# interactiveaudiolab/ppgs

Measured on AMD Instinct MI355X. Metric: PPG frames/sec (whole node), mel repr, batch=32x1000 frames, higher is better.
Workload: dtype bf16; 1 GPU; configs[1]: mel representation, batch=32 x 1000 frames per GPU, audio resident in HBM -> (32,40,1000) fp32 posteriors in HBM; batch=32, frames=1000, per_gpu_batches=1, parallelism=utterance-sharded x1, no data-path collective

## Files before the change

### ppgs_amd/csrc/ppg_frontend.hip

```cpp
#include "ppg_lds.h"
#include "ppg_launch.h"

#include <hip/hip_fp16.h>

namespace {

constexpr int NFFT = 1024;
constexpr int HOP = 160;
constexpr int NBINS = 513;
constexpr int NMELS = 80;
constexpr int PADR = (NFFT - HOP) / 2;
constexpr int FPB = ppg::kFrontendFrames;
constexpr int SEG = NFFT + (FPB - 1) * HOP;
constexpr int BUF = NFFT + NFFT / 16;
constexpr int MSEG = ppg::kMelSegment;
constexpr int NS = ppg::kMelSteps;
constexpr int MROW = 1088;
__device__ __forceinline__ int sigma(int c) { return (0x6c >> (2 * c)) & 3; }

constexpr int OFF_TW = 0;
constexpr int SEGP = (SEG + 255) / 256 * 256;
constexpr int OFF_SEG = OFF_TW + 64 * 8;
constexpr int OFF_FFT = OFF_SEG + 2 * SEGP * 4;
constexpr int OFF_MAG = OFF_FFT + 4 * BUF * 8;
constexpr int LDS_BYTES = OFF_MAG + FPB * MROW;
constexpr int TEAMS = 2;
constexpr int CU_LDS_BYTES = 163840;
static_assert(2 * LDS_BYTES <= CU_LDS_BYTES && LDS_BYTES % 16 == 0, "two teams per CU; a two-team workgroup = the CU's LDS");
static_assert(OFF_MAG % 16 == 0 && MROW % 16 == 0, "fragment reads are 16-byte aligned");

typedef float cplx __attribute__((ext_vector_type(2)));
__device__ __forceinline__ cplx cadd(cplx a, cplx b) { return a + b; }
__device__ __forceinline__ cplx csub(cplx a, cplx b) { return a - b; }
__device__ __forceinline__ cplx cadd_mi(cplx a, cplx b) {
    cplx r;
    asm("v_pk_add_f32 %0, %1, %2 op_sel:[1,0] op_sel_hi:[0,1] neg_hi:[1,0]" : "=v"(r) : "v"(b), "v"(a));
    return r;
}
__device__ __forceinline__ cplx csub_mi(cplx a, cplx b) {
    cplx r;
    asm("v_pk_add_f32 %0, %1, %2 op_sel:[1,0] op_sel_hi:[0,1] neg_lo:[1,0]" : "=v"(r) : "v"(b), "v"(a));
    return r;
}
__device__ __forceinline__ cplx cmul(cplx a, cplx w) {
    cplx t, r;
    asm("v_pk_mul_f32 %0, %1, %2 op_sel:[0,0] op_sel_hi:[0,1]" : "=v"(t) : "v"(a), "v"(w));
    asm("v_fma_f32 %0, -%1, %2, %3" : "=v"(r.x) : "v"(a.y), "v"(w.y), "v"(t.x));
    asm("v_fma_f32 %0, %1, %2, %3" : "=v"(r.y) : "v"(a.y), "v"(w.x), "v"(t.y));
    return r;
}

template <bool CMI = false>
__device__ __forceinline__ void radix4(cplx& A, cplx& B, cplx& C, cplx& D) {
    const cplx apc = CMI ? cadd_mi(A, C) : cadd(A, C), amc = CMI ? csub_mi(A, C) : csub(A, C);
    const cplx bpd = cadd(B, D), bmd = csub(B, D);
    A = cadd(apc, bpd);
    B = cadd_mi(amc, bmd);
    C = csub(apc, bpd);
    D = csub_mi(amc, bmd);
}

template <int M>
__device__ __forceinline__ cplx w16() {
    constexpr float c1 = 0.92387953251128674f, s1 = 0.38268343236508977f, r = 0.70710678118654752f;
    if constexpr (M == 1) return cplx{c1, -s1};
    else if constexpr (M == 2) return cplx{r, -r};
    else if constexpr (M == 3) return cplx{s1, -c1};
    else if constexpr (M == 6) return cplx{-r, -r};
    else { static_assert(M == 9, "exponent"); return cplx{-c1, s1}; }
}

__device__ __forceinline__ void dft16(cplx (&x)[16]) {
#pragma unroll
    for (int r = 0; r < 4; ++r) radix4(x[r], x[r + 4], x[r + 8], x[r + 12]);
    x[5] = cmul(x[5], w16<1>());  x[9] = cmul(x[9], w16<2>());   x[13] = cmul(x[13], w16<3>());
    x[6] = cmul(x[6], w16<2>());   x[14] = cmul(x[14], w16<6>());
    x[7] = cmul(x[7], w16<3>());  x[11] = cmul(x[11], w16<6>()); x[15] = cmul(x[15], w16<9>());
    radix4(x[0], x[1], x[2], x[3]);
    radix4(x[4], x[5], x[6], x[7]);
    radix4<true>(x[8], x[9], x[10], x[11]);
    radix4(x[12], x[13], x[14], x[15]);
    cplx t;
#define PPG_SWAP(a, b) t = x[a]; x[a] = x[b]; x[b] = t;
    PPG_SWAP(1, 4) PPG_SWAP(2, 8) PPG_SWAP(3, 12) PPG_SWAP(6, 9) PPG_SWAP(7, 13) PPG_SWAP(11, 14)
#undef PPG_SWAP
}

__device__ __forceinline__ int pad(int i) { return i + (i >> 4); }

__device__ __forceinline__ void wave_sync() {
    asm volatile("s_waitcnt lgkmcnt(0)" ::: "memory");
    __builtin_amdgcn_fence(__ATOMIC_ACQ_REL, "wavefront");
    __builtin_amdgcn_wave_barrier();
}

template <bool SPEC, class SRC>
__device__ __forceinline__ void frontend_body(
    const ppg::FrontendTables& tb, const SRC& src, int total_groups, int wide_ok, __half* __restrict__ spec, __half* __restrict__ mel)
{
    extern __shared__ __attribute__((aligned(16))) char smem_all[];
    const int team = TEAMS == 1 ? 0 : __builtin_amdgcn_readfirstlane((int)(threadIdx.x >> 8));
    char* smem = smem_all + team * LDS_BYTES;
    cplx* tw = reinterpret_cast<cplx*>(smem + OFF_TW);
    float* seg0 = reinterpret_cast<float*>(smem + OFF_SEG);

    const int tid = threadIdx.x & 255;
    const int lane = tid & 63;
    const int wave = __builtin_amdgcn_readfirstlane(tid >> 6);
    cplx* buf = reinterpret_cast<cplx*>(smem + OFF_FFT) + wave * BUF;

    if (tid < 64) { const float2 w = tb.twiddle[16 * tid]; tw[tid] = cplx{w.x, w.y}; }
    reinterpret_cast<uint32_t*>(smem + OFF_MAG + (tid >> 4) * MROW + 1024)[tid & 15] = 0u;

    float hreg[16];
    cplx t1[16];
#pragma unroll
    for (int j = 0; j < 16; ++j) hreg[j] = tb.hann[lane + 64 * j];
#pragma unroll
    for (int k = 1; k < 16; ++k) { const float2 w = tb.twiddle[lane * k]; t1[k] = cplx{w.x, w.y}; }

    int step_frag[NS], step_off[NS], step_block[NS];
#pragma unroll
    for (int i = 0; i < NS; ++i) {
        const int4 e = tb.mel_prog[wave * NS + i];
        step_frag[i] = __builtin_amdgcn_readfirstlane(e.x);
        step_off[i] = __builtin_amdgcn_readfirstlane(e.y);
        step_block[i] = __builtin_amdgcn_readfirstlane(e.z);
    }

    auto stage = [&](int grp, int into) { src.stage(tb, grp, into, seg0, wave, lane, wide_ok); };
    const int stride = TEAMS * gridDim.x;
    const int first_group = TEAMS * blockIdx.x + team;
    if (first_group < total_groups) stage(first_group, 0);
    asm volatile("s_waitcnt vmcnt(0)" ::: "memory");

#ifdef PPG_FE_TIMING
    int stamp_group = 0;
    auto stamp = [&](int k) {
        if (tb.dbg && blockIdx.x == 0 && lane == 0 && stamp_group == 2) tb.dbg[wave * 16 + k] = __builtin_amdgcn_s_memtime();
    };
#else
    auto stamp = [&](int) {};
#endif
    int half = 0;
    const int trips = (total_groups - TEAMS * (int)blockIdx.x + stride - 1) / stride;
    int grp = first_group;
    for (int trip = 0; trip < trips; ++trip, grp += stride, half ^= 1) {
        const bool active = grp < total_groups;
        int b, f0, frames;
        src.group(grp, active, b, f0, frames);
        const float* seg = seg0 + half * SEGP;
        int pitch = src.pitch(frames);
        asm volatile("" : "+s"(pitch));
#ifdef PPG_FE_TIMING
        ++stamp_group;
#endif
        stamp(0);
        __syncthreads();
        stamp(1);

        auto transform = [&](const int j, const bool verify = false) {
            const int fa = f0 + 2 * j;
            if (fa >= frames) return;
            cplx x[16];
            {
                const float* sa = seg + (2 * j) * HOP + lane;
#pragma unroll
                for (int i = 0; i < 16; ++i) {
                    x[i] = cplx{sa[64 * i], sa[64 * i + HOP]} * hreg[i];
                }
                dft16(x);
#pragma unroll
                for (int k = 1; k < 16; ++k) x[k] = cmul(x[k], t1[k]);
#pragma unroll
                for (int k = 0; k < 16; ++k) buf[17 * lane + k] = x[k];
            }
            wave_sync();
            const int p0 = lane + (lane >> 4);
            {
#pragma unroll
                for (int i = 0; i < 16; ++i) x[i] = buf[p0 + 68 * i];
                dft16(x);
                const int p = lane >> 4, q = lane & 15;
#pragma unroll
                for (int k = 1; k < 16; ++k) x[k] = cmul(x[k], tw[p * k]);
                cplx* dst = buf + q + 272 * p;
#pragma unroll
                for (int k = 0; k < 16; ++k) dst[17 * k] = x[k];
            }
            wave_sync();
#pragma unroll
            for (int m = 0; m < 4; ++m) {
                cplx* z = buf + p0 + 68 * m;
                cplx A = z[0], B = z[272], C = z[544], D = z[816];
                radix4(A, B, C, D);
                z[0] = A; z[272] = B; z[544] = C; z[816] = D;
            }
            wave_sync();
            const int nb = (NFFT - lane) + ((NFFT - lane) >> 4);
            const int odd = lane & 1;
            const int row = j + 8 * odd;
            char* wdst = smem + OFF_MAG + row * MROW + ((((lane >> 3) ^ sigma(row >> 2)) << 2) + ((lane >> 1) & 3)) * 4;
            const uint32_t sel = odd ? 0x07060302u : 0x01000504u;
            auto split_bin = [&](int r, __half& ha, __half& hb) {
                const int k = lane + 64 * r;
                const cplx zk = buf[p0 + 68 * r];
                const cplx zn = buf[(r == 0 && lane == 0) ? 0 : nb - 68 * r];
                const float ar = 0.5f * (zk.x + zn.x), ai = 0.5f * (zk.y - zn.y);
                const float br = 0.5f * (zk.y + zn.y), bi = -0.5f * (zk.x - zn.x);
                ha = __float2half_rn(__builtin_amdgcn_sqrtf(ar * ar + ai * ai + 1e-6f));
                hb = __float2half_rn(__builtin_amdgcn_sqrtf(br * br + bi * bi + 1e-6f));
                if constexpr (SPEC) {
                    if (verify) return;
                    spec[(uint32_t)(b * NBINS + k) * (uint32_t)pitch + (uint32_t)fa] = ha;
                    if (fa + 1 < frames) spec[(uint32_t)(b * NBINS + k) * (uint32_t)pitch + (uint32_t)fa + 1u] = hb;
                }
            };
#pragma unroll
            for (int r = 0; r < 8; ++r) {
                __half ha, hb;
                split_bin(r, ha, hb);
                const uint32_t pk = (uint32_t)__half_as_ushort(ha) | ((uint32_t)__half_as_ushort(hb) << 16);
                const uint32_t other = (uint32_t)__builtin_amdgcn_mov_dpp((int)pk, 0xB1, 0xf, 0xf, true);
                const uint32_t val = __builtin_amdgcn_perm(pk, other, sel);
                *reinterpret_cast<uint32_t*>(wdst + 128 * r) = val;
            }
            if (verify) return;
            if (lane == 0) {
                __half ha, hb;
                split_bin(8, ha, hb);
                *reinterpret_cast<uint32_t*>(smem + OFF_MAG + j * MROW + ((64 ^ sigma(j >> 2)) << 4)) = __half_as_ushort(ha);
                *reinterpret_cast<uint32_t*>(smem + OFF_MAG + (j + 8) * MROW + ((64 ^ sigma((j + 8) >> 2)) << 4)) = __half_as_ushort(hb);
            }
        };

        transform(wave);
        stamp(2);
        if (!(wide_ok & 4) && grp + stride < total_groups) stage(grp + stride, half ^ 1);
        stamp(3);
        transform(wave + 4);
        stamp(4);
        u32x4 whi[NS], wlo[NS];
        asm volatile("s_waitcnt vmcnt(0)" ::: "memory");
        if (mel) {
            uint32_t loff = lane * 16;
            asm volatile("" : "+v"(loff));
#pragma unroll
            for (int i = 0; i < NS; ++i) {
                const char* src = reinterpret_cast<const char*>(tb.mel_img) + (size_t)step_frag[i] * 1024;
                whi[i] = *reinterpret_cast<const u32x4*>(src + loff);
                wlo[i] = *reinterpret_cast<const u32x4*>(src + 1024 + loff);
            }
        }
        __syncthreads();
        stamp(5);
        if (mel) {
            const int n = lane & 15, g = lane >> 4;
            const char* brow = smem + OFF_MAG + n * MROW + ((g ^ sigma(n >> 2)) << 4);
            f32x4 acc = {0.f, 0.f, 0.f, 0.f};
            const int frame = f0 + (n < 8 ? 2 * n : 2 * (n - 8) + 1);
#pragma unroll
            for (int i = 0; i < NS; ++i) {
                const u32x4 bfi = *reinterpret_cast<const u32x4*>(brow + step_off[i]);
                PrecF16::mma(acc, whi[i], bfi);
                PrecF16::mma(acc, wlo[i], bfi);
                const int block = step_block[i];
                if ((i == MSEG - 1 || i == NS - 1) && block >= 0) {
                    if (frame < frames) {
#pragma unroll
                        for (int e = 0; e < 4; ++e) {
                            const int m = 16 * block + 4 * g + e;
                            mel[(uint32_t)(b * NMELS + m) * (uint32_t)pitch + (uint32_t)frame] =
                                __float2half_rn(logf(fmaxf(acc[e] * (1.0f / 65536.0f), 1e-5f)));
                        }
                    }
                    acc = f32x4{0.f, 0.f, 0.f, 0.f};
                }
            }
        }
        stamp(6);
        if (wide_ok & 4) {
            __syncthreads();
            if (grp + stride < total_groups) stage(grp + stride, half ^ 1);
            asm volatile("s_waitcnt vmcnt(0)" ::: "memory");
        }
        if constexpr (SRC::kCarry) { if (active) src.carry_forward(grp, tid); }
    }
}

struct BatchSource {
    static constexpr bool kCarry = false;
    const float* __restrict__ audio;
    int samples, frames, groups_per_row;
    __device__ __forceinline__ void group(int grp, bool active, int& b, int& f0, int& nframes) const {
        b = active ? grp / groups_per_row : 0;
        f0 = active ? (grp - b * groups_per_row) * FPB : frames;
        nframes = frames;
    }
    __device__ __forceinline__ int pitch(int nframes) const { return nframes; }
    __device__ __forceinline__ void stage(const ppg::FrontendTables& tb, int grp, int into, float* seg0, int wave, int lane, int wide_ok) const {
        const int b = grp / groups_per_row;
        const int f0 = (grp - b * groups_per_row) * FPB;
        const float* arow = audio + (size_t)b * samples;
        const uint32_t dst = lds_addr(seg0) + into * (SEGP * 4);
        const int first = f0 * HOP - PADR;
        if ((wide_ok & 1) && first >= 0 && first + SEGP <= samples) {
#pragma unroll
            for (int j = 0; j < (SEGP / 256 + 3) / 4; ++j) {
                const int piece = wave + 4 * j;
                if (piece >= SEGP / 256) break;
                glds16_saddr(reinterpret_cast<const char*>(arow + first), (uint32_t)(piece * 1024 + lane * 16), dst + piece * 1024);
            }
            return;
        }
#pragma unroll 2
        for (int piece = wave; piece < SEGP / 64; piece += 4) {
            int src = first + piece * 64 + lane;
            if (src < 0) src = -src;
            if (src >= samples) src = 2 * (samples - 1) - src;
            const float* p = (src >= 0 && src < samples) ? arow + src : tb.hann;
            asm volatile("s_mov_b32 m0, %1\n\ts_nop 0\n\tglobal_load_lds_dword %0, off"
                         :: "v"(p), "s"(__builtin_amdgcn_readfirstlane(dst + piece * 256)) : "memory", "m0");
        }
    }
};

template <bool SPEC>
__global__ __launch_bounds__(256 * TEAMS, 2 / TEAMS) void frontend_kernel(
    ppg::FrontendTables tb, const float* __restrict__ audio, int samples, int frames,
    int groups_per_row, int total_groups, int wide_ok, __half* __restrict__ spec, __half* __restrict__ mel)
{
    frontend_body<SPEC>(tb, BatchSource{audio, samples, frames, groups_per_row}, total_groups, wide_ok, spec, mel);
}

struct StreamSource {
    static constexpr bool kCarry = true;
    ppg::FrontendStreamArgs a;
    __device__ __forceinline__ void group(int grp, bool active, int& b, int& f0, int& nframes) const {
        const int l = active ? grp / a.groups_per_item : 0;
        nframes = active ? a.item[l].frames : 0;
        f0 = active ? (grp - l * a.groups_per_item) * FPB : 0;
        b = a.item0 + l;
    }
    __device__ __forceinline__ int pitch(int) const { return a.out_pitch; }
    __device__ __forceinline__ const float* sample(const ppg::FrontendStreamItem& it, int l, int pos) const {
        return pos < it.split ? a.carry + ((size_t)(2 * (a.item0 + l) + it.cur) * a.cap + (pos - it.cbase))
                              : a.chunk + ((size_t)(a.item0 + l) * a.chunk_pitch + (pos - it.split));
    }
    __device__ __forceinline__ void stage(const ppg::FrontendTables& tb, int grp, int into, float* seg0, int wave, int lane, int) const {
        const int l = grp / a.groups_per_item;
        const int f0 = (grp - l * a.groups_per_item) * FPB;
        const ppg::FrontendStreamItem it = a.item[l];
        if (f0 >= it.frames) return;
        const uint32_t dst = lds_addr(seg0) + into * (SEGP * 4);
        const int first = f0 * HOP - PADR;
#pragma unroll 2
        for (int piece = wave; piece < SEGP / 64; piece += 4) {
            int pos = first + piece * 64 + lane;
            if (pos < it.lo) pos = 2 * it.lo - pos;
            if (pos >= it.hi) pos = 2 * (it.hi - 1) - pos;
            const float* p = (pos >= it.cbase && pos < it.hi) ? sample(it, l, pos) : tb.hann;
            asm volatile("s_mov_b32 m0, %1\n\ts_nop 0\n\tglobal_load_lds_dword %0, off"
                         :: "v"(p), "s"(__builtin_amdgcn_readfirstlane(dst + piece * 256)) : "memory", "m0");
        }
    }
    __device__ __forceinline__ void carry_forward(int grp, int tid) const {
        const int l = grp / a.groups_per_item;
        if (grp != l * a.groups_per_item) return;
        const ppg::FrontendStreamItem it = a.item[l];
        float* next = a.carry + (size_t)(2 * (a.item0 + l) + (it.cur ^ 1)) * a.cap;
        for (int pos = it.keep + tid; pos < it.hi; pos += 256) next[pos - it.keep] = *sample(it, l, pos);
    }
};

__global__ __launch_bounds__(256 * TEAMS, 2 / TEAMS) void frontend_stream_kernel(
    ppg::FrontendTables tb, StreamSource src, int total_groups, __half* __restrict__ mel)
{
    frontend_body<false>(tb, src, total_groups, 0, nullptr, mel);
}

}

namespace ppg {

hipError_t launch_frontend(const FrontendTables& tb, const float* audio, int batch, int samples,
                           void* spec, void* mel, hipStream_t s) {
    const int frames = samples / HOP;
    const int groups_per_row = (frames + FPB - 1) / FPB;
    if (mel && (!tb.mel_img || !tb.mel_prog)) return hipErrorInvalidValue;
    if ((double)batch * NBINS * frames >= 4294967296.0) return hipErrorInvalidValue;
    const int total = groups_per_row * batch;
    static LdsLimit limit[2];
    const void* kernel = spec ? reinterpret_cast<const void*>(frontend_kernel<true>) : reinterpret_cast<const void*>(frontend_kernel<false>);
    const hipError_t e = limit[spec != nullptr].ensure(kernel, CU_LDS_BYTES);
    if (e != hipSuccess) return e;
    static int slots = 0;
    if (slots == 0) {
        int dev = 0, cus = 0;
        if (hipGetDevice(&dev) != hipSuccess ||
            hipDeviceGetAttribute(&cus, hipDeviceAttributeMultiprocessorCount, dev) != hipSuccess || cus <= 0)
            cus = 256;
        slots = 2 * cus;
    }
    const int rounds = (total + slots - 1) / slots;
    const int teams = (total + rounds - 1) / rounds;
    const int grid = (teams + TEAMS - 1) / TEAMS;
    int wide_ok = (reinterpret_cast<uintptr_t>(audio) % 16 == 0 && samples % 4 == 0) ? 1 : 0;
    size_t lds_bytes = TEAMS == 2 ? CU_LDS_BYTES : LDS_BYTES;
    static const int fe_debug = env_experiment("PPGS_AMD_FE_DEBUG", 0);
    if (fe_debug & 1) wide_ok = 0;
    if (fe_debug & 4) wide_ok |= 4;
    if (fe_debug & 16) lds_bytes = TEAMS * LDS_BYTES;
    if (spec)
        hipLaunchKernelGGL(frontend_kernel<true>, dim3(grid), dim3(256 * TEAMS), lds_bytes, s, tb, audio, samples, frames,
                           groups_per_row, total, wide_ok, reinterpret_cast<__half*>(spec), reinterpret_cast<__half*>(mel));
    else
        hipLaunchKernelGGL(frontend_kernel<false>, dim3(grid), dim3(256 * TEAMS), lds_bytes, s, tb, audio, samples, frames,
                           groups_per_row, total, wide_ok, reinterpret_cast<__half*>(spec), reinterpret_cast<__half*>(mel));
    return hipGetLastError();
}

hipError_t launch_frontend_stream(const FrontendTables& tb, const FrontendStreamArgs& args, int items, void* mel, hipStream_t s) {
    if (!tb.mel_img || !tb.mel_prog || items <= 0 || items > kFrontendStreamItems || args.groups_per_item <= 0)
        return hipErrorInvalidValue;
    if ((double)(args.item0 + items) * NMELS * args.out_pitch >= 4294967296.0) return hipErrorInvalidValue;
    static LdsLimit limit;
    const hipError_t e = limit.ensure(reinterpret_cast<const void*>(frontend_stream_kernel), CU_LDS_BYTES);
    if (e != hipSuccess) return e;
    static int slots = 0;
    if (slots == 0) {
        int dev = 0, cus = 0;
        if (hipGetDevice(&dev) != hipSuccess ||
            hipDeviceGetAttribute(&cus, hipDeviceAttributeMultiprocessorCount, dev) != hipSuccess || cus <= 0)
            cus = 256;
        slots = 2 * cus;
    }
    const int total = args.groups_per_item * items;
    const int rounds = (total + slots - 1) / slots;
    const int teams = (total + rounds - 1) / rounds;
    const int grid = (teams + TEAMS - 1) / TEAMS;
    hipLaunchKernelGGL(frontend_stream_kernel, dim3(grid), dim3(256 * TEAMS), CU_LDS_BYTES, s, tb, StreamSource{args}, total,
                       reinterpret_cast<__half*>(mel));
    return hipGetLastError();
}

}
```

Before: 48.58 million frames/s.

## Restructure 1024-point FFT as 32x32 with half-wave transforms and bpermute spectrum split

Replaces the three-pass 16x16x4 FFT per wave with a two-pass 32x32 decomposition in which each half-wave (32 lanes) transforms one frame pair. The transpose goes through a float-wide padded LDS buffer in two halves (real, then imaginary), which halves the FFT scratch footprint. The conjugate-symmetric partner bins now come from ds_bpermute instead of LDS reads. Hann and twiddle values are loaded from global memory inside the loop rather than kept in registers, and the mel frame ordering changes to match the new row layout. This should cut LDS passes and barriers, but it raises register pressure with 32-element complex arrays and adds global reads on every trip.

```diff
diff --git a/ppgs_amd/csrc/ppg_frontend.hip b/ppgs_amd/csrc/ppg_frontend.hip
--- a/ppgs_amd/csrc/ppg_frontend.hip
+++ b/ppgs_amd/csrc/ppg_frontend.hip
@@ -2,6 +2,8 @@
 #include "ppg_launch.h"
 
 #include <hip/hip_fp16.h>
+
+#include <utility>
 
 namespace {
 
@@ -12,17 +14,17 @@
 constexpr int PADR = (NFFT - HOP) / 2;
 constexpr int FPB = ppg::kFrontendFrames;
 constexpr int SEG = NFFT + (FPB - 1) * HOP;
-constexpr int BUF = NFFT + NFFT / 16;
+constexpr int XROW = 33;
+constexpr int BUF = 2 * 32 * XROW;
 constexpr int MSEG = ppg::kMelSegment;
 constexpr int NS = ppg::kMelSteps;
 constexpr int MROW = 1088;
 __device__ __forceinline__ int sigma(int c) { return (0x6c >> (2 * c)) & 3; }
 
-constexpr int OFF_TW = 0;
 constexpr int SEGP = (SEG + 255) / 256 * 256;
-constexpr int OFF_SEG = OFF_TW + 64 * 8;
+constexpr int OFF_SEG = 0;
 constexpr int OFF_FFT = OFF_SEG + 2 * SEGP * 4;
-constexpr int OFF_MAG = OFF_FFT + 4 * BUF * 8;
+constexpr int OFF_MAG = OFF_FFT + 4 * BUF * 4;
 constexpr int LDS_BYTES = OFF_MAG + FPB * MROW;
 constexpr int TEAMS = 2;
 constexpr int CU_LDS_BYTES = 163840;
@@ -47,6 +49,13 @@
     asm("v_pk_mul_f32 %0, %1, %2 op_sel:[0,0] op_sel_hi:[0,1]" : "=v"(t) : "v"(a), "v"(w));
     asm("v_fma_f32 %0, -%1, %2, %3" : "=v"(r.x) : "v"(a.y), "v"(w.y), "v"(t.x));
     asm("v_fma_f32 %0, %1, %2, %3" : "=v"(r.y) : "v"(a.y), "v"(w.x), "v"(t.y));
+    return r;
+}
+__device__ __forceinline__ cplx cmul_conj(cplx a, cplx w) {
+    cplx t, r;
+    asm("v_pk_mul_f32 %0, %1, %2 op_sel:[0,0] op_sel_hi:[0,1]" : "=v"(t) : "v"(a), "v"(w));
+    asm("v_fma_f32 %0, %1, %2, %3" : "=v"(r.x) : "v"(a.y), "v"(w.y), "v"(t.x));
+    asm("v_fma_f32 %0, %1, %2, -%3" : "=v"(r.y) : "v"(a.y), "v"(w.x), "v"(t.y));
     return r;
 }
 
@@ -86,7 +95,30 @@
 #undef PPG_SWAP
 }
 
-__device__ __forceinline__ int pad(int i) { return i + (i >> 4); }
+template <int M>
+__device__ __forceinline__ cplx w32() {
+    constexpr float c[8] = {1.f, 0.98078528040323043f, 0.92387953251128674f, 0.83146961230254524f,
+                            0.70710678118654752f, 0.55557023301960218f, 0.38268343236508977f, 0.19509032201612825f};
+    static_assert(M >= 1 && M <= 7, "exponent");
+    return cplx{c[M], -c[8 - M]};
+}
+
+__device__ __forceinline__ void dft32(cplx (&x)[32]) {
+    cplx e[16], o[16];
+#pragma unroll
+    for (int i = 0; i < 16; ++i) { e[i] = x[2 * i]; o[i] = x[2 * i + 1]; }
+    dft16(e);
+    __builtin_amdgcn_sched_barrier(0);
+    dft16(o);
+    __builtin_amdgcn_sched_barrier(0);
+    auto fly = [&](auto kc) {
+        constexpr int k = decltype(kc)::value;
+        if constexpr (k % 8 != 0) o[k] = cmul(o[k], w32<k % 8>());
+        if constexpr (k < 8) { x[k] = cadd(e[k], o[k]); x[k + 16] = csub(e[k], o[k]); }
+        else { x[k] = cadd_mi(e[k], o[k]); x[k + 16] = csub_mi(e[k], o[k]); }
+    };
+    [&]<int... K>(std::integer_sequence<int, K...>) { (fly(std::integral_constant<int, K>{}), ...); }(std::make_integer_sequence<int, 16>{});
+}
 
 __device__ __forceinline__ void wave_sync() {
     asm volatile("s_waitcnt lgkmcnt(0)" ::: "memory");
@@ -101,23 +133,15 @@
     extern __shared__ __attribute__((aligned(16))) char smem_all[];
     const int team = TEAMS == 1 ? 0 : __builtin_amdgcn_readfirstlane((int)(threadIdx.x >> 8));
     char* smem = smem_all + team * LDS_BYTES;
-    cplx* tw = reinterpret_cast<cplx*>(smem + OFF_TW);
     float* seg0 = reinterpret_cast<float*>(smem + OFF_SEG);
 
     const int tid = threadIdx.x & 255;
     const int lane = tid & 63;
     const int wave = __builtin_amdgcn_readfirstlane(tid >> 6);
-    cplx* buf = reinterpret_cast<cplx*>(smem + OFF_FFT) + wave * BUF;
-
-    if (tid < 64) { const float2 w = tb.twiddle[16 * tid]; tw[tid] = cplx{w.x, w.y}; }
+    const int q = lane & 31, hw = lane >> 5;
+    float* xbuf = reinterpret_cast<float*>(smem + OFF_FFT) + wave * BUF + hw * (32 * XROW);
+
     reinterpret_cast<uint32_t*>(smem + OFF_MAG + (tid >> 4) * MROW + 1024)[tid & 15] = 0u;
-
-    float hreg[16];
-    cplx t1[16];
-#pragma unroll
-    for (int j = 0; j < 16; ++j) hreg[j] = tb.hann[lane + 64 * j];
-#pragma unroll
-    for (int k = 1; k < 16; ++k) { const float2 w = tb.twiddle[lane * k]; t1[k] = cplx{w.x, w.y}; }
 
     int step_frag[NS], step_off[NS], step_block[NS];
 #pragma unroll
@@ -159,86 +183,89 @@
         __syncthreads();
         stamp(1);
 
-        auto transform = [&](const int j, const bool verify = false) {
-            const int fa = f0 + 2 * j;
-            if (fa >= frames) return;
-            cplx x[16];
+
+        const bool work = f0 + 4 * wave < frames;
+        const int j = 2 * wave + hw;
+        const int fa = f0 + 2 * j;
+        cplx x[32];
+        if (work) {
             {
-                const float* sa = seg + (2 * j) * HOP + lane;
-#pragma unroll
-                for (int i = 0; i < 16; ++i) {
-                    x[i] = cplx{sa[64 * i], sa[64 * i + HOP]} * hreg[i];
-                }
-                dft16(x);
-#pragma unroll
-                for (int k = 1; k < 16; ++k) x[k] = cmul(x[k], t1[k]);
-#pragma unroll
-                for (int k = 0; k < 16; ++k) buf[17 * lane + k] = x[k];
-            }
-            wave_sync();
-            const int p0 = lane + (lane >> 4);
+                uint32_t qoff = q;
+                asm volatile("" : "+v"(qoff));
+                const float* hw_ = tb.hann + qoff;
+                const float* sa = seg + (2 * j) * HOP + q;
+#pragma unroll
+                for (int i = 0; i < 32; ++i) x[i] = cplx{sa[32 * i], sa[32 * i + HOP]} * hw_[32 * i];
+                cplx t1[17];
+#pragma unroll
+                for (int k = 1; k <= 16; ++k) { const float2 w = tb.twiddle[qoff * k]; t1[k] = cplx{w.x, w.y}; }
+                __builtin_amdgcn_sched_barrier(0);
+                dft32(x);
+                __builtin_amdgcn_sched_barrier(0);
+#pragma unroll
+                for (int k = 1; k < 32; ++k) x[k] = k <= 16 ? cmul(x[k], t1[k]) : cmul_conj(x[k], t1[32 - k]);
+            }
+        }
+        stamp(2);
+        if (!(wide_ok & 4) && grp + stride < total_groups) stage(grp + stride, half ^ 1);
+        if (work) {
             {
-#pragma unroll
-                for (int i = 0; i < 16; ++i) x[i] = buf[p0 + 68 * i];
-                dft16(x);
-                const int p = lane >> 4, q = lane & 15;
-#pragma unroll
-                for (int k = 1; k < 16; ++k) x[k] = cmul(x[k], tw[p * k]);
-                cplx* dst = buf + q + 272 * p;
-#pragma unroll
-                for (int k = 0; k < 16; ++k) dst[17 * k] = x[k];
-            }
-            wave_sync();
-#pragma unroll
-            for (int m = 0; m < 4; ++m) {
-                cplx* z = buf + p0 + 68 * m;
-                cplx A = z[0], B = z[272], C = z[544], D = z[816];
-                radix4(A, B, C, D);
-                z[0] = A; z[272] = B; z[544] = C; z[816] = D;
-            }
-            wave_sync();
-            const int nb = (NFFT - lane) + ((NFFT - lane) >> 4);
+                float* col = xbuf + XROW * q;
+                const float* rowp = xbuf + q;
+                float re[32];
+#pragma unroll
+                for (int k = 0; k < 32; ++k) col[k] = x[k].x;
+                wave_sync();
+#pragma unroll
+                for (int i = 0; i < 32; ++i) re[i] = rowp[XROW * i];
+                wave_sync();
+#pragma unroll
+                for (int k = 0; k < 32; ++k) col[k] = x[k].y;
+                wave_sync();
+#pragma unroll
+                for (int i = 0; i < 32; ++i) x[i] = cplx{re[i], rowp[XROW * i]};
+            }
+            stamp(3);
+            __builtin_amdgcn_sched_barrier(0);
+            dft32(x);
+            __builtin_amdgcn_sched_barrier(0);
             const int odd = lane & 1;
-            const int row = j + 8 * odd;
-            char* wdst = smem + OFF_MAG + row * MROW + ((((lane >> 3) ^ sigma(row >> 2)) << 2) + ((lane >> 1) & 3)) * 4;
+            const int row = 2 * j + odd;
+            char* wdst = smem + OFF_MAG + row * MROW + ((((q >> 3) ^ sigma(row >> 2)) << 2) + ((q >> 1) & 3)) * 4;
             const uint32_t sel = odd ? 0x07060302u : 0x01000504u;
-            auto split_bin = [&](int r, __half& ha, __half& hb) {
-                const int k = lane + 64 * r;
-                const cplx zk = buf[p0 + 68 * r];
-                const cplx zn = buf[(r == 0 && lane == 0) ? 0 : nb - 68 * r];
+            const int partner = ((lane & 32) | ((32 - q) & 31)) << 2;
+            auto split_bin = [&](int k, cplx zk, cplx zn, __half& ha, __half& hb) {
                 const float ar = 0.5f * (zk.x + zn.x), ai = 0.5f * (zk.y - zn.y);
                 const float br = 0.5f * (zk.y + zn.y), bi = -0.5f * (zk.x - zn.x);
                 ha = __float2half_rn(__builtin_amdgcn_sqrtf(ar * ar + ai * ai + 1e-6f));
                 hb = __float2half_rn(__builtin_amdgcn_sqrtf(br * br + bi * bi + 1e-6f));
                 if constexpr (SPEC) {
-                    if (verify) return;
-                    spec[(uint32_t)(b * NBINS + k) * (uint32_t)pitch + (uint32_t)fa] = ha;
+                    if (fa < frames) spec[(uint32_t)(b * NBINS + k) * (uint32_t)pitch + (uint32_t)fa] = ha;
                     if (fa + 1 < frames) spec[(uint32_t)(b * NBINS + k) * (uint32_t)pitch + (uint32_t)fa + 1u] = hb;
                 }
             };
 #pragma unroll
-            for (int r = 0; r < 8; ++r) {
+            for (int k2 = 0; k2 < 16; ++k2) {
+                const cplx mine = (q == 0 || q >= 17) ? x[(32 - k2) & 31] : x[31 - k2];
+                cplx zn;
+                zn.x = __int_as_float(__builtin_amdgcn_ds_bpermute(partner, __float_as_int(mine.x)));
+                zn.y = __int_as_float(__builtin_amdgcn_ds_bpermute(partner, __float_as_int(mine.y)));
                 __half ha, hb;
-                split_bin(r, ha, hb);
+                split_bin(q + 32 * k2, q >= 17 ? x[k2 + 1] : x[k2], zn, ha, hb);
                 const uint32_t pk = (uint32_t)__half_as_ushort(ha) | ((uint32_t)__half_as_ushort(hb) << 16);
                 const uint32_t other = (uint32_t)__builtin_amdgcn_mov_dpp((int)pk, 0xB1, 0xf, 0xf, true);
                 const uint32_t val = __builtin_amdgcn_perm(pk, other, sel);
-                *reinterpret_cast<uint32_t*>(wdst + 128 * r) = val;
-            }
-            if (verify) return;
-            if (lane == 0) {
+                *reinterpret_cast<uint32_t*>(wdst + 64 * k2) = val;
+                if (k2 % 4 == 3) __builtin_amdgcn_sched_barrier(0);
+            }
+            if (q == 0) {
                 __half ha, hb;
-                split_bin(8, ha, hb);
-                *reinterpret_cast<uint32_t*>(smem + OFF_MAG + j * MROW + ((64 ^ sigma(j >> 2)) << 4)) = __half_as_ushort(ha);
-                *reinterpret_cast<uint32_t*>(smem + OFF_MAG + (j + 8) * MROW + ((64 ^ sigma((j + 8) >> 2)) << 4)) = __half_as_ushort(hb);
-            }
-        };
-
-        transform(wave);
-        stamp(2);
-        if (!(wide_ok & 4) && grp + stride < total_groups) stage(grp + stride, half ^ 1);
-        stamp(3);
-        transform(wave + 4);
+                split_bin(512, x[16], x[16], ha, hb);
+                const int s4 = (64 ^ sigma(j >> 1)) << 4;
+                *reinterpret_cast<uint32_t*>(smem + OFF_MAG + (2 * j) * MROW + s4) = __half_as_ushort(ha);
+                *reinterpret_cast<uint32_t*>(smem + OFF_MAG + (2 * j + 1) * MROW + s4) = __half_as_ushort(hb);
+            }
+        }
         stamp(4);
         u32x4 whi[NS], wlo[NS];
         asm volatile("s_waitcnt vmcnt(0)" ::: "memory");
@@ -258,7 +285,7 @@
             const int n = lane & 15, g = lane >> 4;
             const char* brow = smem + OFF_MAG + n * MROW + ((g ^ sigma(n >> 2)) << 4);
             f32x4 acc = {0.f, 0.f, 0.f, 0.f};
-            const int frame = f0 + (n < 8 ? 2 * n : 2 * (n - 8) + 1);
+            const int frame = f0 + n;
 #pragma unroll
             for (int i = 0; i < NS; ++i) {
                 const u32x4 bfi = *reinterpret_cast<const u32x4*>(brow + step_off[i]);
```

Measured after the change: 48.49 million frames/s. About the same (-0.2%).
